# jasperlinthorst/reveal

Hardware: AMD Instinct MI355X
Metric: Mbp/s indexed+MUM-anchored (reveal rem) (higher is better)
Workload: dtype int32

## Files before the change

reveal_amd/csrc/rv_prims.hip:

```cpp
#include "rv_common.h"
#include <string.h>

namespace {

constexpr int SCAN_THREADS = 256;
constexpr int SCAN_ITEMS   = 8;
constexpr int SCAN_TILE    = SCAN_THREADS * SCAN_ITEMS;

template <class T> struct OpSum {
    __device__ static T id() { return (T)0; }
    __device__ static T f(T a, T b) { return a + b; }
};
template <class T> struct OpMax {
    __device__ static T id() { return (T)0; }
    __device__ static T f(T a, T b) { return a > b ? a : b; }
};

template <class T> __device__ inline T shfl_up_t(T v, int d) { return __shfl_up(v, d, 64); }
template <> __device__ inline u64 shfl_up_t<u64>(u64 v, int d) {
    u32 lo = __shfl_up((u32)v, d, 64), hi = __shfl_up((u32)(v >> 32), d, 64);
    return ((u64)hi << 32) | lo;
}

template <class T, class Op>
__device__ inline T block_exclusive(T x, T *lds , T *total) {
    const int lane = threadIdx.x & 63, w = threadIdx.x >> 6;
    T inc = x;
#pragma unroll
    for (int d = 1; d < 64; d <<= 1) {
        T t = shfl_up_t<T>(inc, d);
        if (lane >= d) inc = Op::f(t, inc);
    }
    T exc = shfl_up_t<T>(inc, 1);
    if (lane == 0) exc = Op::id();
    if (lane == 63) lds[w] = inc;
    __syncthreads();
    T base = Op::id(), tot = Op::id();
#pragma unroll
    for (int k = 0; k < SCAN_THREADS / 64; k++) {
        T v = lds[k];
        if (k < w) base = Op::f(base, v);
        tot = Op::f(tot, v);
    }
    __syncthreads();
    *total = tot;
    return Op::f(base, exc);
}

template <class T, class Op>
__global__ __launch_bounds__(SCAN_THREADS) void k_tile_reduce(const T *__restrict__ in, T *__restrict__ totals, int64_t n) {
    __shared__ T lds[4];
    const int64_t base = (int64_t)blockIdx.x * SCAN_TILE + (int64_t)threadIdx.x * SCAN_ITEMS;
    T acc = Op::id();
    if (base + SCAN_ITEMS <= n) {
        T v[SCAN_ITEMS];
        __builtin_memcpy(v, in + base, sizeof v);
#pragma unroll
        for (int i = 0; i < SCAN_ITEMS; i++) acc = Op::f(acc, v[i]);
    } else {
#pragma unroll
        for (int i = 0; i < SCAN_ITEMS; i++)
            if (base + i < n) acc = Op::f(acc, in[base + i]);
    }
    T tot;
    (void)block_exclusive<T, Op>(acc, lds, &tot);
    if (threadIdx.x == 0) totals[blockIdx.x] = tot;
}

template <class T, class Op, bool INCL>
__global__ __launch_bounds__(SCAN_THREADS) void k_tile_scan(const T *in, T *out, const T *__restrict__ tile_prefix, int64_t n) {
    __shared__ T lds[4];
    const int64_t base = (int64_t)blockIdx.x * SCAN_TILE + (int64_t)threadIdx.x * SCAN_ITEMS;
    T v[SCAN_ITEMS];
    const bool whole = base + SCAN_ITEMS <= n;
    if (whole) __builtin_memcpy(v, in + base, sizeof v);
    else {
#pragma unroll
        for (int i = 0; i < SCAN_ITEMS; i++) v[i] = (base + i < n) ? in[base + i] : Op::id();
    }
    T acc = Op::id();
#pragma unroll
    for (int i = 0; i < SCAN_ITEMS; i++) acc = Op::f(acc, v[i]);
    T tot;
    T pre = block_exclusive<T, Op>(acc, lds, &tot);
    if (tile_prefix) pre = Op::f(tile_prefix[blockIdx.x], pre);
    if (whole) {
        T o[SCAN_ITEMS];
#pragma unroll
        for (int i = 0; i < SCAN_ITEMS; i++) { const T nx = Op::f(pre, v[i]); o[i] = INCL ? nx : pre; pre = nx; }
        __builtin_memcpy(out + base, o, sizeof o);
        return;
    }
#pragma unroll
    for (int i = 0; i < SCAN_ITEMS; i++) {
        T nx = Op::f(pre, v[i]);
        if (base + i < n) out[base + i] = INCL ? nx : pre;
        pre = nx;
    }
}

template <class T, class Op, bool INCL>
int scan_rec(Workspace &ws, const T *in, T *out, int64_t n, int level) {
    if (n <= 0) return 0;
    const int64_t nt = ceil_div(n, SCAN_TILE);
    if (nt == 1) {
        hipLaunchKernelGGL((k_tile_scan<T, Op, INCL>), dim3(1), dim3(SCAN_THREADS), 0, ws.stream, in, out, (const T *)nullptr, n);
        RV_LAUNCH_CHECK();
        return 0;
    }
    if (level >= 4) { rv_set_error("scan: too many levels"); return -1; }
    RV_TRY(ws.scan_tmp[level].reserve((size_t)nt * sizeof(T)));
    T *tot = ws.scan_tmp[level].as<T>();
    hipLaunchKernelGGL((k_tile_reduce<T, Op>), dim3((unsigned)nt), dim3(SCAN_THREADS), 0, ws.stream, in, tot, n);
    RV_LAUNCH_CHECK();
    RV_TRY((scan_rec<T, Op, false>(ws, tot, tot, nt, level + 1)));
    hipLaunchKernelGGL((k_tile_scan<T, Op, INCL>), dim3((unsigned)nt), dim3(SCAN_THREADS), 0, ws.stream, in, out, (const T *)tot, n);
    RV_LAUNCH_CHECK();
    return 0;
}

}

int rv_exclusive_sum_u32(Workspace &ws, const u32 *in, u32 *out, int64_t n) { return scan_rec<u32, OpSum<u32>, false>(ws, in, out, n, 0); }
int rv_exclusive_sum_u64(Workspace &ws, const u64 *in, u64 *out, int64_t n) { return scan_rec<u64, OpSum<u64>, false>(ws, in, out, n, 0); }
int rv_inclusive_max_u32(Workspace &ws, const u32 *in, u32 *out, int64_t n) { return scan_rec<u32, OpMax<u32>, true>(ws, in, out, n, 0); }
int rv_inclusive_max_u64(Workspace &ws, const u64 *in, u64 *out, int64_t n) { return scan_rec<u64, OpMax<u64>, true>(ws, in, out, n, 0); }

namespace {

#ifndef RV_RS_THREADS
#define RV_RS_THREADS 256
#endif
constexpr int RS_THREADS = RV_RS_THREADS;
#ifndef RV_RS_ITEMS
#define RV_RS_ITEMS 16
#endif
constexpr int RS_ITEMS   = RV_RS_ITEMS;
constexpr int RS_TILE    = RS_THREADS * RS_ITEMS;
constexpr int RS_WAVES   = RS_THREADS / 64;

constexpr unsigned RS_XCDS = 8;
template <bool XCD> __device__ inline u32 rs_tile_of(u32 nb) {
    if (!XCD) return blockIdx.x;
    const u32 chunk = (nb + RS_XCDS - 1) / RS_XCDS;
    return (blockIdx.x % RS_XCDS) * chunk + blockIdx.x / RS_XCDS;
}

template <int BITS, bool XCD>
__global__ __launch_bounds__(RS_THREADS) void k_rs_hist(const u64 *__restrict__ keys, int64_t n, int shift, u32 dmask, u32 *__restrict__ blockhist, u32 nblocks) {
    constexpr int NB = 1 << BITS;
    __shared__ u32 h[NB];
    const u32 tile = rs_tile_of<XCD>(nblocks);
    if (tile >= nblocks) return;
    for (int k = threadIdx.x; k < NB; k += RS_THREADS) h[k] = 0;
    __syncthreads();
    const int64_t base = (int64_t)tile * RS_TILE;
    u64 key[RS_ITEMS];
#pragma unroll
    for (int r = 0; r < RS_ITEMS; r++) {
        const int64_t i = base + (int64_t)r * RS_THREADS + threadIdx.x;
        key[r] = i < n ? keys[i] : 0ull;
    }
#pragma unroll
    for (int r = 0; r < RS_ITEMS; r++) {
        const int64_t i = base + (int64_t)r * RS_THREADS + threadIdx.x;
        if (i < n) atomicAdd(&h[(u32)(key[r] >> shift) & dmask], 1u);
    }
    __syncthreads();
    for (int k = threadIdx.x; k < NB; k += RS_THREADS) blockhist[(size_t)k * nblocks + tile] = h[k];
}

template <bool XCD>
__global__ __launch_bounds__(RS_THREADS) void k_rs_hist_bytes(const uint8_t *__restrict__ digits, int64_t n, u32 *__restrict__ blockhist, u32 nblocks) {
    static_assert(RS_ITEMS == 16, "sixteen digit bytes per thread");
    __shared__ u32 h[256];
    const u32 tile = rs_tile_of<XCD>(nblocks);
    if (tile >= nblocks) return;
    h[threadIdx.x] = 0;
    __syncthreads();
    const int64_t i0 = (int64_t)tile * RS_TILE + (int64_t)threadIdx.x * 16;
    if (i0 + 16 <= n) {
        const uint4 v = *reinterpret_cast<const uint4 *>(digits + i0);
        const u32 w[4] = {v.x, v.y, v.z, v.w};
#pragma unroll
        for (int k = 0; k < 4; k++)
#pragma unroll
            for (int b = 0; b < 4; b++) atomicAdd(&h[(w[k] >> (8 * b)) & 255u], 1u);
    } else {
        for (int64_t i = i0; i < n && i < i0 + 16; i++) atomicAdd(&h[digits[i]], 1u);
    }
    __syncthreads();
    blockhist[(size_t)threadIdx.x * nblocks + tile] = h[threadIdx.x];
}

template <class V, int BITS, bool XCD, class CNT>
__global__ __launch_bounds__(RS_THREADS) void k_rs_scatter(const u64 *__restrict__ kin, const V *__restrict__ vin,
                                                            u64 *__restrict__ kout, V *__restrict__ vout, int64_t n, int shift, u32 dmask,
                                                            const u32 *__restrict__ blockoff, u32 nblocks, uint8_t *__restrict__ dnext, int nshift, u32 nmask) {
    constexpr int NB = 1 << BITS;
    constexpr int BPT = NB / RS_THREADS;
    static_assert(NB % RS_THREADS == 0 && RS_TILE < 65536, "bins per thread, 16-bit counters");
    __shared__ CNT cnt[RS_WAVES][NB];
    __shared__ u32 gbase[NB];
    __shared__ CNT dstart[NB];
    __shared__ u32 wtot[RS_WAVES];
    __shared__ u64 skey[RS_TILE];
    __shared__ V sval[RS_TILE];
    const u32 tile = rs_tile_of<XCD>(nblocks);
    if (tile >= nblocks) return;
    const int lane = threadIdx.x & 63, w = threadIdx.x >> 6;
    for (int k = threadIdx.x; k < RS_WAVES * NB; k += RS_THREADS) (&cnt[0][0])[k] = 0;
    for (int k = threadIdx.x; k < NB; k += RS_THREADS) gbase[k] = blockoff[(size_t)k * nblocks + tile];
    __syncthreads();

    const int64_t wbase = (int64_t)tile * RS_TILE + (int64_t)w * (64 * RS_ITEMS);
    u64 key[RS_ITEMS];
    V val[RS_ITEMS];
    u32 rnk[RS_ITEMS];
    const u64 lt = (lane == 0) ? 0ull : (~0ull >> (64 - lane));
#pragma unroll
    for (int r = 0; r < RS_ITEMS; r++) {
        const int64_t i = wbase + (int64_t)r * 64 + lane;
        key[r] = i < n ? kin[i] : ~0ull;
    }
#pragma unroll
    for (int r = 0; r < RS_ITEMS; r++) {
        const int64_t i = wbase + (int64_t)r * 64 + lane;
        val[r] = i < n ? vin[i] : V(0);
    }
#pragma unroll
    for (int r = 0; r < RS_ITEMS; r++) {
        const int64_t i = wbase + (int64_t)r * 64 + lane;
        const bool valid = i < n;
        const u32 d = (u32)(key[r] >> shift) & dmask;
        u64 peers = __ballot(valid);
#pragma unroll
        for (int b = 0; b < BITS; b++) {
            const bool bit = (d >> b) & 1u;
            const u64 bal = __ballot(bit);
            peers &= bit ? bal : ~bal;
        }
        const u32 below = (u32)__popcll(peers & lt);
        const u32 old = cnt[w][d];
        __builtin_amdgcn_wave_barrier();
        if (valid && below == 0) cnt[w][d] = (CNT)(old + (u32)__popcll(peers));
        __builtin_amdgcn_wave_barrier();
        rnk[r] = old + below;
    }
    __syncthreads();
    u32 tot[BPT], mytot = 0;
#pragma unroll
    for (int b = 0; b < BPT; b++) {
        const int d = threadIdx.x * BPT + b;
        u32 run = 0;
#pragma unroll
        for (int k = 0; k < RS_WAVES; k++) { const u32 c = cnt[k][d]; cnt[k][d] = (CNT)run; run += c; }
        tot[b] = run; mytot += run;
    }
    {
        u32 inc = mytot;
#pragma unroll
        for (int dd = 1; dd < 64; dd <<= 1) { const u32 t = __shfl_up(inc, dd, 64); if (lane >= dd) inc += t; }
        if (lane == 63) wtot[w] = inc;
        __syncthreads();
        u32 before = inc - mytot;
#pragma unroll
        for (int k = 0; k < RS_WAVES; k++) if (k < w) before += wtot[k];
#pragma unroll
        for (int b = 0; b < BPT; b++) { dstart[threadIdx.x * BPT + b] = (CNT)before; before += tot[b]; }
    }
    __syncthreads();
#pragma unroll
    for (int r = 0; r < RS_ITEMS; r++) {
        const int64_t i = wbase + (int64_t)r * 64 + lane;
        if (i < n) {
            const u32 d = (u32)(key[r] >> shift) & dmask;
            const u32 li = (u32)dstart[d] + (u32)cnt[w][d] + rnk[r];
            skey[li] = key[r];
            sval[li] = val[r];
        }
    }
    __syncthreads();
    const int64_t tbase = (int64_t)tile * RS_TILE;
    const u32 nvalid = (u32)((n - tbase) < (int64_t)RS_TILE ? (n - tbase) : (int64_t)RS_TILE);
    for (u32 li = threadIdx.x; li < nvalid; li += RS_THREADS) {
        const u64 k = skey[li];
        const u32 d = (u32)(k >> shift) & dmask;
        const size_t dst = (size_t)gbase[d] + (li - (u32)dstart[d]);
        kout[dst] = k;
        vout[dst] = sval[li];
        if (dnext) dnext[dst] = (uint8_t)((u32)(k >> nshift) & nmask);
    }
}

template <class V, int BITS, bool XCD, class CNT>
static void rs_scatter_launch(hipStream_t q, u32 nb, const u64 *ki, const V *vi, u64 *ko, V *vo, int64_t n, int shift, u32 dmask, const u32 *bh,
                              uint8_t *dnext, int nshift, u32 nmask) {
    const u32 grid = XCD ? RS_XCDS * ((nb + RS_XCDS - 1) / RS_XCDS) : nb;
    hipLaunchKernelGGL((k_rs_scatter<V, BITS, XCD, CNT>), dim3(grid), dim3(RS_THREADS), 0, q, ki, vi, ko, vo, n, shift, dmask, bh, nb, dnext, nshift, nmask);
}

}

int rv_radix_passes(const Workspace &ws, int nbits) {
    const int w = ws.opt.rs_bits == 10 ? 10 : 8;
    return nbits <= 0 ? 0 : (nbits + w - 1) / w;
}

static bool rs_digit_bytes(const Workspace &ws, int64_t n, int bit_lo, int bit_hi) {
    return ws.opt.rs_bits != 10 && !ws.opt.rs_no_digit_bytes && n > 1 && n >= ((int64_t)1 << 20) && n < ((int64_t)1 << 32) && bit_hi - bit_lo > 8;
}
uint8_t *rv_radix_first_digits(Workspace &ws, int64_t n, int bit_lo, int bit_hi) {
    if (!rs_digit_bytes(ws, n, bit_lo, bit_hi) || ws.rs_digits.reserve((size_t)n + 64)) return nullptr;
    return ws.rs_digits.as<uint8_t>();
}

template <class V>
int rv_radix_sort_pairs(Workspace &ws, u64 *k0, V *v0, u64 *k1, V *v1, int64_t n, int bit_lo, int bit_hi, int *result_in_1, bool first_digits) {
    *result_in_1 = 0;
    if (n <= 1 || bit_hi <= bit_lo) return 0;
    if (n >= ((int64_t)1 << 32)) { rv_set_error("radix sort: n >= 2^32 not supported"); return -1; }
    const int width = ws.opt.rs_bits == 10 ? 10 : 8;
    const bool xcd = ws.opt.rs_xcd != 0, c16 = ws.opt.rs_cnt16 != 0;
    const u32 nb = (u32)ceil_div(n, RS_TILE);
    RV_TRY(ws.rs_hist.reserve(((size_t)1 << width) * nb * sizeof(u32)));
    u32 *bh = ws.rs_hist.as<u32>();
    const bool bytes = rs_digit_bytes(ws, n, bit_lo, bit_hi);
    if (first_digits && (!bytes || ws.rs_digits.cap < (size_t)n + 64)) { rv_set_error("radix sort: first digits announced but the byte path is off"); return -1; }
    if (bytes) RV_TRY(ws.rs_digits.reserve((size_t)n + 64));
    uint8_t *dig = bytes ? ws.rs_digits.as<uint8_t>() : nullptr;
    bool have_digits = first_digits;
    u64 *ki = k0, *ko = k1;
    V *vi = v0, *vo = v1;
    int flip = 0;
    for (int shift = bit_lo; shift < bit_hi; shift += width) {
        const int wbits = bit_hi - shift < width ? bit_hi - shift : width;
        const u32 dmask = (1u << wbits) - 1u;
        int pid = ws.prof_begin(8 , (have_digits ? 1.0 : 8.0) * (double)n);
        const u32 hgrid = xcd ? RS_XCDS * ((nb + RS_XCDS - 1) / RS_XCDS) : nb;
        if (have_digits) {
            if (xcd) hipLaunchKernelGGL((k_rs_hist_bytes<true>), dim3(hgrid), dim3(RS_THREADS), 0, ws.stream, (const uint8_t *)dig, n, bh, nb);
            else hipLaunchKernelGGL((k_rs_hist_bytes<false>), dim3(hgrid), dim3(RS_THREADS), 0, ws.stream, (const uint8_t *)dig, n, bh, nb);
        } else if (width == 10) { if (xcd) hipLaunchKernelGGL((k_rs_hist<10, true>), dim3(hgrid), dim3(RS_THREADS), 0, ws.stream, (const u64 *)ki, n, shift, dmask, bh, nb);
                           else hipLaunchKernelGGL((k_rs_hist<10, false>), dim3(hgrid), dim3(RS_THREADS), 0, ws.stream, (const u64 *)ki, n, shift, dmask, bh, nb); }
        else             { if (xcd) hipLaunchKernelGGL((k_rs_hist<8, true>), dim3(hgrid), dim3(RS_THREADS), 0, ws.stream, (const u64 *)ki, n, shift, dmask, bh, nb);
                           else hipLaunchKernelGGL((k_rs_hist<8, false>), dim3(hgrid), dim3(RS_THREADS), 0, ws.stream, (const u64 *)ki, n, shift, dmask, bh, nb); }
        RV_LAUNCH_CHECK();
        ws.prof_end(pid);
        RV_TRY(rv_exclusive_sum_u32(ws, bh, bh, ((int64_t)1 << width) * nb));
        const int nshift = shift + width;
        const bool more = nshift < bit_hi;
        const u32 nmask = more ? ((1u << (bit_hi - nshift < width ? bit_hi - nshift : width)) - 1u) : 0u;
        uint8_t *dn = (bytes && more) ? dig : nullptr;
        pid = ws.prof_begin(7 , (2.0 * (8.0 + sizeof(V)) + (dn ? 1.0 : 0.0)) * (double)n);
#define RS_GO(B_, X_, C_) rs_scatter_launch<V, B_, X_, C_>(ws.stream, nb, (const u64 *)ki, (const V *)vi, ko, vo, n, shift, dmask, (const u32 *)bh, dn, nshift, nmask)
        if (width == 10) { if (xcd) { if (c16) RS_GO(10, true, uint16_t); else RS_GO(10, true, u32); } else { if (c16) RS_GO(10, false, uint16_t); else RS_GO(10, false, u32); } }
        else             { if (xcd) { if (c16) RS_GO(8, true, uint16_t); else RS_GO(8, true, u32); } else { if (c16) RS_GO(8, false, uint16_t); else RS_GO(8, false, u32); } }
#undef RS_GO
        RV_LAUNCH_CHECK();
        ws.prof_end(pid);
        have_digits = dn != nullptr;
        u64 *tk = ki; ki = ko; ko = tk;
        V *tv = vi; vi = vo; vo = tv;
        flip ^= 1;
    }
    *result_in_1 = flip;
    return 0;
}

__global__ __launch_bounds__(256) void k_h2d_copy(const uint4 *__restrict__ src, uint4 *__restrict__ dst, size_t n16) {
    for (size_t i = (size_t)blockIdx.x * 256 + threadIdx.x; i < n16; i += (size_t)gridDim.x * 256) dst[i] = src[i];
}
int rv_read_back(Workspace &ws, void *dst, const void *dsrc, size_t bytes) {
    RV_TRY(ws.hpin.reserve(bytes < 4096 ? 4096 : bytes));
    if (!ws.ev_rb) RV_HIP(hipEventCreateWithFlags(&ws.ev_rb, hipEventDisableTiming));
    RV_HIP(hipMemcpyAsync(ws.hpin.p, dsrc, bytes, hipMemcpyDeviceToHost, ws.stream));
    RV_HIP(hipEventRecord(ws.ev_rb, ws.stream));
    const hipError_t e = rv_event_wait(ws.ev_rb);
    if (e != hipSuccess) { rv_set_error("rv_read_back: %s", hipGetErrorString(e)); return -1; }
    memcpy(dst, ws.hpin.p, bytes);
    return 0;
}

int rv_read_back2(Workspace &ws, void *dst_a, const void *dsrc_a, size_t bytes_a, void *dst_b, const void *dsrc_b, size_t bytes_b) {
    const size_t off = (bytes_a + 63) & ~(size_t)63;
    RV_TRY(ws.hpin.reserve(off + bytes_b < 4096 ? 4096 : off + bytes_b));
    if (!ws.ev_rb) RV_HIP(hipEventCreateWithFlags(&ws.ev_rb, hipEventDisableTiming));
    RV_HIP(hipMemcpyAsync(ws.hpin.p, dsrc_a, bytes_a, hipMemcpyDeviceToHost, ws.stream));
    RV_HIP(hipMemcpyAsync((uint8_t *)ws.hpin.p + off, dsrc_b, bytes_b, hipMemcpyDeviceToHost, ws.stream));
    RV_HIP(hipEventRecord(ws.ev_rb, ws.stream));
    const hipError_t e = rv_event_wait(ws.ev_rb);
    if (e != hipSuccess) { rv_set_error("rv_read_back2: %s", hipGetErrorString(e)); return -1; }
    memcpy(dst_a, ws.hpin.p, bytes_a);
    memcpy(dst_b, (const uint8_t *)ws.hpin.p + off, bytes_b);
    return 0;
}

int rv_h2d_copy(Workspace &ws, const void *pinned_src, void *dst, size_t bytes) {
    const size_t n16 = (bytes + 15) / 16;
    if (n16 == 0) return 0;
    size_t blocks = (n16 + 255) / 256;
    if (blocks > 512) blocks = 512;
    hipLaunchKernelGGL(k_h2d_copy, dim3((unsigned)blocks), dim3(256), 0, ws.stream, (const uint4 *)pinned_src, (uint4 *)dst, n16);
    RV_LAUNCH_CHECK();
    return 0;
}

template int rv_radix_sort_pairs<u32>(Workspace &, u64 *, u32 *, u64 *, u32 *, int64_t, int, int, int *, bool);
template int rv_radix_sort_pairs<u64>(Workspace &, u64 *, u64 *, u64 *, u64 *, int64_t, int, int, int *, bool);
```

Measured before the change: 25090.

## Alias radix-scatter value staging onto key LDS buffer and restructure ranking

The onesweep-style radix scatter kernel now stages values in the same shared buffer as the keys, writing them out in a second phase after the keys have been emitted. This drops the separate sval array, and launch bounds plus an explicit dynamic LDS allocation are set to pin occupancy for the 8-bit variant. The per-wave digit ranking is rewritten with 32-bit halves and bitop3 masking. Rank and digit are packed into one register, local indices are packed in pairs, and full tiles are specialised to skip bounds checks. The cost is an extra barrier round and values being written out separately from keys, which may reduce write coalescing overlap.

```diff
diff --git a/reveal_amd/csrc/rv_prims.hip b/reveal_amd/csrc/rv_prims.hip
--- a/reveal_amd/csrc/rv_prims.hip
+++ b/reveal_amd/csrc/rv_prims.hip
@@ -1,5 +1,6 @@
 #include "rv_common.h"
 #include <string.h>
+#include <type_traits>
 
 namespace {
 
@@ -193,59 +194,61 @@
     blockhist[(size_t)threadIdx.x * nblocks + tile] = h[threadIdx.x];
 }
 
+constexpr unsigned RS_LDS_HOLD = 8192;
 template <class V, int BITS, bool XCD, class CNT>
-__global__ __launch_bounds__(RS_THREADS) void k_rs_scatter(const u64 *__restrict__ kin, const V *__restrict__ vin,
+__global__ __launch_bounds__(RS_THREADS, BITS == 8 ? 4 : 1) void k_rs_scatter(const u64 *__restrict__ kin, const V *__restrict__ vin,
                                                             u64 *__restrict__ kout, V *__restrict__ vout, int64_t n, int shift, u32 dmask,
                                                             const u32 *__restrict__ blockoff, u32 nblocks, uint8_t *__restrict__ dnext, int nshift, u32 nmask) {
     constexpr int NB = 1 << BITS;
     constexpr int BPT = NB / RS_THREADS;
-    static_assert(NB % RS_THREADS == 0 && RS_TILE < 65536, "bins per thread, 16-bit counters");
+    static_assert(NB % RS_THREADS == 0 && RS_TILE < 65536 && RS_ITEMS % 2 == 0, "bins per thread, 16-bit counters and local indices");
+    static_assert(sizeof(V) <= sizeof(u64), "the values are staged where the keys were");
     __shared__ CNT cnt[RS_WAVES][NB];
     __shared__ u32 gbase[NB];
     __shared__ CNT dstart[NB];
     __shared__ u32 wtot[RS_WAVES];
     __shared__ u64 skey[RS_TILE];
-    __shared__ V sval[RS_TILE];
+    static_assert(BITS != 8 || sizeof cnt + sizeof gbase + sizeof dstart + sizeof wtot + sizeof skey <= 40 * 1024, "the 8-bit kernel's own arrays: 40 KiB at most");
+    V *const sval = reinterpret_cast<V *>(skey);
     const u32 tile = rs_tile_of<XCD>(nblocks);
     if (tile >= nblocks) return;
-    const int lane = threadIdx.x & 63, w = threadIdx.x >> 6;
+    const int lane = threadIdx.x & 63, w = __builtin_amdgcn_readfirstlane(threadIdx.x >> 6);
     for (int k = threadIdx.x; k < RS_WAVES * NB; k += RS_THREADS) (&cnt[0][0])[k] = 0;
     for (int k = threadIdx.x; k < NB; k += RS_THREADS) gbase[k] = blockoff[(size_t)k * nblocks + tile];
     __syncthreads();
 
-    const int64_t wbase = (int64_t)tile * RS_TILE + (int64_t)w * (64 * RS_ITEMS);
+    const int64_t tbase = (int64_t)tile * RS_TILE;
+    const u32 nvalid = (u32)((n - tbase) < (int64_t)RS_TILE ? (n - tbase) : (int64_t)RS_TILE);
+    const u32 wfirst = (u32)w * (64 * RS_ITEMS) + (u32)lane;
+    const u64 *const kw = kin + tbase + w * (64 * RS_ITEMS);
+    const V *const vw = vin + tbase + w * (64 * RS_ITEMS);
     u64 key[RS_ITEMS];
     V val[RS_ITEMS];
-    u32 rnk[RS_ITEMS];
-    const u64 lt = (lane == 0) ? 0ull : (~0ull >> (64 - lane));
+    u32 rd[RS_ITEMS];
+    u32 lidx[RS_ITEMS / 2];
+    const u32 lt_lo = lane >= 32 ? ~0u : ((1u << lane) - 1u), lt_hi = lane > 32 ? ((1u << (lane - 32)) - 1u) : 0u;
+#pragma unroll
+    for (int r = 0; r < RS_ITEMS; r++) key[r] = wfirst + 64u * r < nvalid ? kw[r * 64 + lane] : ~0ull;
+#pragma unroll
+    for (int r = 0; r < RS_ITEMS; r++) val[r] = wfirst + 64u * r < nvalid ? vw[r * 64 + lane] : V(0);
 #pragma unroll
     for (int r = 0; r < RS_ITEMS; r++) {
-        const int64_t i = wbase + (int64_t)r * 64 + lane;
-        key[r] = i < n ? kin[i] : ~0ull;
-    }
-#pragma unroll
-    for (int r = 0; r < RS_ITEMS; r++) {
-        const int64_t i = wbase + (int64_t)r * 64 + lane;
-        val[r] = i < n ? vin[i] : V(0);
-    }
-#pragma unroll
-    for (int r = 0; r < RS_ITEMS; r++) {
-        const int64_t i = wbase + (int64_t)r * 64 + lane;
-        const bool valid = i < n;
         const u32 d = (u32)(key[r] >> shift) & dmask;
-        u64 peers = __ballot(valid);
+        u32 plo = ~0u, phi = ~0u;
 #pragma unroll
         for (int b = 0; b < BITS; b++) {
-            const bool bit = (d >> b) & 1u;
-            const u64 bal = __ballot(bit);
-            peers &= bit ? bal : ~bal;
+            int m = (int)(d << (31 - b)) >> 31;
+            asm("" : "+v"(m));
+            const u64 bal = __ballot(m != 0);
+            plo = __builtin_amdgcn_bitop3_b32(plo, (u32)bal, (u32)m, 0x90);
+            phi = __builtin_amdgcn_bitop3_b32(phi, (u32)(bal >> 32), (u32)m, 0x90);
         }
-        const u32 below = (u32)__popcll(peers & lt);
+        const u32 below = (u32)__popc(plo & lt_lo) + (u32)__popc(phi & lt_hi);
         const u32 old = cnt[w][d];
         __builtin_amdgcn_wave_barrier();
-        if (valid && below == 0) cnt[w][d] = (CNT)(old + (u32)__popcll(peers));
+        if (below == 0) cnt[w][d] = (CNT)(old + (u32)__popc(plo) + (u32)__popc(phi));
         __builtin_amdgcn_wave_barrier();
-        rnk[r] = old + below;
+        rd[r] = (old + below) | (d << 16);
     }
     __syncthreads();
     u32 tot[BPT], mytot = 0;
@@ -272,32 +275,45 @@
     __syncthreads();
 #pragma unroll
     for (int r = 0; r < RS_ITEMS; r++) {
-        const int64_t i = wbase + (int64_t)r * 64 + lane;
-        if (i < n) {
-            const u32 d = (u32)(key[r] >> shift) & dmask;
-            const u32 li = (u32)dstart[d] + (u32)cnt[w][d] + rnk[r];
-            skey[li] = key[r];
-            sval[li] = val[r];
+        const u32 d = rd[r] >> 16;
+        const u32 li = (u32)dstart[d] + (u32)cnt[w][d] + (rd[r] & 0xFFFFu);
+        skey[li] = key[r];
+        if (r & 1) lidx[r >> 1] |= li << 16; else lidx[r >> 1] = li;
+    }
+    __syncthreads();
+    auto out = [&](auto whole) {
+        constexpr bool WHOLE = decltype(whole)::value;
+        u32 dst[RS_ITEMS];
+#pragma unroll
+        for (int j = 0; j < RS_ITEMS; j++) {
+            const u32 li = (u32)j * RS_THREADS + threadIdx.x;
+            dst[j] = 0;
+            if (WHOLE || li < nvalid) {
+                const u64 k = skey[li];
+                const u32 d = (u32)(k >> shift) & dmask;
+                dst[j] = gbase[d] + (li - (u32)dstart[d]);
+                kout[dst[j]] = k;
+                if (dnext) dnext[dst[j]] = (uint8_t)((u32)(k >> nshift) & nmask);
+            }
         }
-    }
-    __syncthreads();
-    const int64_t tbase = (int64_t)tile * RS_TILE;
-    const u32 nvalid = (u32)((n - tbase) < (int64_t)RS_TILE ? (n - tbase) : (int64_t)RS_TILE);
-    for (u32 li = threadIdx.x; li < nvalid; li += RS_THREADS) {
-        const u64 k = skey[li];
-        const u32 d = (u32)(k >> shift) & dmask;
-        const size_t dst = (size_t)gbase[d] + (li - (u32)dstart[d]);
-        kout[dst] = k;
-        vout[dst] = sval[li];
-        if (dnext) dnext[dst] = (uint8_t)((u32)(k >> nshift) & nmask);
-    }
+        __syncthreads();
+#pragma unroll
+        for (int r = 0; r < RS_ITEMS; r++) sval[(lidx[r >> 1] >> (16 * (r & 1))) & 0xFFFFu] = val[r];
+        __syncthreads();
+#pragma unroll
+        for (int j = 0; j < RS_ITEMS; j++) {
+            const u32 li = (u32)j * RS_THREADS + threadIdx.x;
+            if (WHOLE || li < nvalid) vout[dst[j]] = sval[li];
+        }
+    };
+    if (nvalid == (u32)RS_TILE) out(std::true_type()); else out(std::false_type());
 }
 
 template <class V, int BITS, bool XCD, class CNT>
 static void rs_scatter_launch(hipStream_t q, u32 nb, const u64 *ki, const V *vi, u64 *ko, V *vo, int64_t n, int shift, u32 dmask, const u32 *bh,
                               uint8_t *dnext, int nshift, u32 nmask) {
     const u32 grid = XCD ? RS_XCDS * ((nb + RS_XCDS - 1) / RS_XCDS) : nb;
-    hipLaunchKernelGGL((k_rs_scatter<V, BITS, XCD, CNT>), dim3(grid), dim3(RS_THREADS), 0, q, ki, vi, ko, vo, n, shift, dmask, bh, nb, dnext, nshift, nmask);
+    hipLaunchKernelGGL((k_rs_scatter<V, BITS, XCD, CNT>), dim3(grid), dim3(RS_THREADS), BITS == 8 ? RS_LDS_HOLD : 0u, q, ki, vi, ko, vo, n, shift, dmask, bh, nb, dnext, nshift, nmask);
 }
 
 }
```

After: 25030. Within noise of the previous version (-0.2%).
